# luotuoqingshan/SDPLRPlus.jl

Hardware: NVIDIA B200
Metric: AL inner iterations per second, MaxCut on a synthetic 10M-vertex power-law graph (rank 10) (higher is better)
Workload: dtype f64

## Files before the change

### sdplrplus.jl_b200/csrc/aop.cu

```cuda
#include <algorithm>
#include "common.cuh"

namespace {

constexpr int TPB = 256;

template <int VEC>
struct Ld;
template <>
struct Ld<1> {
    typedef double T;
    static __device__ __forceinline__ T ld(const double *p) { return __ldg(p); }
    static __device__ __forceinline__ double dot(T a, T b) { return a * b; }
};
template <>
struct Ld<2> {
    typedef double2 T;
    static __device__ __forceinline__ T ld(const double *p) { return ldg2(p); }
    static __device__ __forceinline__ double dot(T a, T b) { return a.x * b.x + a.y * b.y; }
};

template <int MODE, int VEC>
__device__ __forceinline__ void entry_accum(const double *__restrict__ U, const double *__restrict__ V, int r, int nv,
                                            int row, int col, int lg, int G, double v2, double &a1, double &a2,
// ... 73 lines not shown
    }
}

template <int MODE, int VEC>
__global__ void __launch_bounds__(TPB) k_A_rowc(long long lo, long long hi, const int *__restrict__ rowc_ptr,
                                                const double *__restrict__ rowc_val,
                                                const double *__restrict__ U, const double *__restrict__ V, int r, int G,
                                                double *__restrict__ out1, double *__restrict__ out2) {
    typedef Ld<VEC> L;
    __shared__ double sh1[TPB], sh2[TPB];
    const int nv = r / VEC;
    const int rpt = TPB / nv;
    const int rl = threadIdx.x / nv, c = threadIdx.x - rl * nv;
    const long long n_rows = hi - lo;
    for (long long t0 = (long long)blockIdx.x * rpt; t0 < n_rows; t0 += (long long)gridDim.x * rpt) {
        const long long i = lo + t0 + rl;
        const bool live = rl < rpt && i < hi;
        double d1 = 0.0, d2 = 0.0;
        int beg = 0, end = 0;
        if (live && c == 0) { beg = rowc_ptr[i]; end = rowc_ptr[i + 1]; }
        if (live) {
            typename L::T a = L::ld(U + (size_t)i * r + c * VEC);
            if (MODE == 0) {
                d1 = L::dot(a, a);
            } else {
                typename L::T b = L::ld(V + (size_t)i * r + c * VEC);
                d1 = L::dot(a, b);
                if (MODE == 2) d2 = L::dot(b, b);
            }
        }
        sh1[threadIdx.x] = d1;
        if (MODE == 2) sh2[threadIdx.x] = d2;
        __syncthreads();
        if (live && c == 0) {
            if (end > beg) {
                double s1 = 0.0, s2 = 0.0;
                for (int k = 0; k < nv; k++) { s1 += sh1[threadIdx.x + k]; if (MODE == 2) s2 += sh2[threadIdx.x + k]; }
                for (int k = beg; k < end; k++) {
                    const double val = rowc_val[k];
                    out1[k] = (MODE == 2 ? 2.0 : 1.0) * val * s1;
                    if (MODE == 2) out2[k] = val * s2;
                }
            }
        }
        __syncthreads();
    }
}

constexpr int kRowcUnroll = 4;
template <int MODE, int VEC>
__global__ void __launch_bounds__(TPB, 4) k_A_rowc_warp(long long lo, long long hi, const int *__restrict__ rowc_ptr,
// ... 8 lines not shown
    const bool act = rl < rpw;
    const long long n_rows = hi - lo;
    const long long per_trip = (long long)rpw * kRowcUnroll;
    const long long warp = (long long)blockIdx.x * (TPB / 32) + (threadIdx.x >> 5);
    const long long n_warps = (long long)gridDim.x * (TPB / 32);
    for (long long t0 = warp * per_trip; t0 < n_rows; t0 += n_warps * per_trip) {
        double d1[kRowcUnroll], d2[kRowcUnroll];
        int beg[kRowcUnroll], end[kRowcUnroll];
        typename L::T a[kRowcUnroll], b[kRowcUnroll];
#pragma unroll
        for (int u = 0; u < kRowcUnroll; u++) {
            const long long i = lo + t0 + (long long)u * rpw + rl;
            const bool live = act && i < hi;
            const long long is = live ? i : hi - 1;
            beg[u] = 0; end[u] = 0;
            if (live && c == 0) { beg[u] = rowc_ptr[i]; end[u] = rowc_ptr[i + 1]; }
            a[u] = L::ld(U + (size_t)is * r + c * VEC);
            if (MODE != 0) b[u] = L::ld(V + (size_t)is * r + c * VEC);
        }
#pragma unroll
        for (int u = 0; u < kRowcUnroll; u++) {
            d2[u] = 0.0;
            if (MODE == 0) {
                d1[u] = L::dot(a[u], a[u]);
            } else {
                d1[u] = L::dot(a[u], b[u]);
                if (MODE == 2) d2[u] = L::dot(b[u], b[u]);
            }
        }
#pragma unroll
        for (int u = 0; u < kRowcUnroll; u++) {
            double s1 = 0.0 + d1[u], s2 = 0.0 + d2[u];
            for (int k = 1; k < nv; k++) {
                s1 += __shfl_down_sync(0xffffffffu, d1[u], k);
                if (MODE == 2) s2 += __shfl_down_sync(0xffffffffu, d2[u], k);
            }
            for (int k = beg[u]; k < end[u]; k++) {
                const double val = rowc_val[k];
                out1[k] = (MODE == 2 ? 2.0 : 1.0) * val * s1;
                if (MODE == 2) out2[k] = val * s2;
            }
        }
    }
}

template <int MODE, int VEC>
__global__ void __launch_bounds__(TPB) k_A_long(const int *__restrict__ chunk_mat, const int *__restrict__ long_mat,
                                                const int *__restrict__ long_chunk_ptr, const int *__restrict__ matptr,
                                                const int *__restrict__ ent_row, const int *__restrict__ ent_col,
                                                const double *__restrict__ ent_two, const double *__restrict__ U,
// ... 80 lines not shown
            double t = 0.0;
            for (unsigned bI = 0; bI < gridDim.x; bI++) t += __ldcg(&part[(size_t)bI * (r * s) + e]);
            out[e] = t;
        }
        if (threadIdx.x == 0) *ticket = 0u;
    }
}

__global__ void k_lr_trace(int r, int s, const double *__restrict__ UB, const double *__restrict__ VB,
                           const double *__restrict__ Dg, double mult, double *__restrict__ out, int gid) {
    double acc[1] = {0.0};
    for (int e = threadIdx.x; e < r * s; e += blockDim.x) acc[0] += UB[e] * VB[e] * Dg[e / r];
    block_sum<1>(acc);
    if (threadIdx.x == 0) out[gid] = acc[0] * mult;
}

int pick_group(int nv) {
    int G = 1;
    while (G < nv && G < 32) G <<= 1;
    return G;
}

template <int MODE>
int32_t run_sparse(sdplrp_handle *h, const double *U, const double *V, double *out1, double *out2, int skip_mat = -1) {
    if (h->nA <= 0) return SDPLRP_OK;
    cudaStream_t st = h->stream;
    const int r = h->r;
    const bool vec2 = (r % 2 == 0);
    const int nv = vec2 ? r / 2 : r;
    const int G = pick_group(nv);
    const int gpb = TPB / G;
    const int grid_short = grid_for(h->nA, gpb, 16 * kNumSM);
    const int lo = (int)h->row_lo, hi = (int)h->row_hi;
    const unsigned char *sdf = h->n_sd > 0 ? h->sd_flag : nullptr;
    if (h->nA - h->n_sd - h->n_long > 0) {
        if (vec2) k_A_short<MODE, 2><<<grid_short, TPB, 0, st>>>((int)h->nA, h->matptr, h->mat_gid, h->ent_row, h->ent_col, h->ent_two, U, V, r, G, out1, out2, lo, hi, skip_mat, sdf);
        else k_A_short<MODE, 1><<<grid_short, TPB, 0, st>>>((int)h->nA, h->matptr, h->mat_gid, h->ent_row, h->ent_col, h->ent_two, U, V, r, G, out1, out2, lo, hi, skip_mat, sdf);
        KLAUNCH(h);
    }
    if (h->n_sd > 0 && nv <= 32 && h->rowc_kernel == 1 && h->world == 1) {
        const int grid_rows = grid_for(h->row_hi - h->row_lo, (TPB / 32) * (32 / nv) * kRowcUnroll, 16 * kNumSM);
        if (vec2) k_A_rowc_warp<MODE, 2><<<grid_rows, TPB, 0, st>>>(h->row_lo, h->row_hi, h->rowc_ptr, h->rowc_val, U, V, r, out1, out2);
        else k_A_rowc_warp<MODE, 1><<<grid_rows, TPB, 0, st>>>(h->row_lo, h->row_hi, h->rowc_ptr, h->rowc_val, U, V, r, out1, out2);
        KLAUNCH(h);
    } else if (h->n_sd > 0) {
        const int grid_rows = grid_for(h->row_hi - h->row_lo, TPB / nv, 16 * kNumSM);
        if (vec2) k_A_rowc<MODE, 2><<<grid_rows, TPB, 0, st>>>(h->row_lo, h->row_hi, h->rowc_ptr, h->rowc_val, U, V, r, G, out1, out2);
        else k_A_rowc<MODE, 1><<<grid_rows, TPB, 0, st>>>(h->row_lo, h->row_hi, h->rowc_ptr, h->rowc_val, U, V, r, G, out1, out2);
        KLAUNCH(h);
    }
    if (h->n_chunks > 0) {
        if (vec2) k_A_long<MODE, 2><<<(int)h->n_chunks, TPB, 0, st>>>(h->chunk_mat, h->long_mat, h->long_chunk_ptr, h->matptr, h->ent_row, h->ent_col, h->ent_two, U, V, r, G, h->chunk_part, lo, hi, skip_mat);
        else k_A_long<MODE, 1><<<(int)h->n_chunks, TPB, 0, st>>>(h->chunk_mat, h->long_mat, h->long_chunk_ptr, h->matptr, h->ent_row, h->ent_col, h->ent_two, U, V, r, G, h->chunk_part, lo, hi, skip_mat);
        KLAUNCH(h);
        k_A_long_combine<MODE><<<(int)h->n_long, TPB, 0, st>>>(h->long_mat, h->long_chunk_ptr, h->mat_gid, h->chunk_part, out1, out2, skip_mat);
        KLAUNCH(h);
    }
    CUDA_TRY(h, cudaGetLastError());
    return SDPLRP_OK;
}

}

int32_t lr_project(sdplrp_handle *h, const LowRank &L, const double *X, double *dst) {
    const int r = h->r;
    if (r > TPB) return fail(h, SDPLRP_ERR_ARG, "low-rank path supports r <= 256");
    const i64 lo = h->row_lo, nloc = h->row_hi - h->row_lo;
    for (i64 k0 = 0; k0 < L.s; k0 += kLrS) {
// ... 40 lines not shown
    }
    CUDA_TRY(h, cudaGetLastError());
    return SDPLRP_OK;
}

int32_t aop_uu_skip(sdplrp_handle *h, const double *U, double *out, bool skip_objective) {
    CUDA_TRY(h, cudaMemsetAsync(out, 0, (size_t)(h->m + 1) * sizeof(double), h->stream));
    SDP_CHECK(run_sparse<0>(h, U, nullptr, out, nullptr, skip_objective ? h->obj_mat : -1));
    return run_lowrank(h, 0, U, nullptr, out, nullptr);
}

int32_t aop_uu(sdplrp_handle *h, const double *U, double *out) { return aop_uu_skip(h, U, out, false); }

int32_t aop_uv(sdplrp_handle *h, const double *U, const double *V, double *out) {
    CUDA_TRY(h, cudaMemsetAsync(out, 0, (size_t)(h->m + 1) * sizeof(double), h->stream));
    SDP_CHECK(run_sparse<1>(h, U, V, out, nullptr));
    return run_lowrank(h, 1, U, V, out, nullptr);
}

int32_t aop_linesearch(sdplrp_handle *h, bool skip_objective) {
    const i64 z0 = h->world == 1 ? h->n_sd : 0;
    CUDA_TRY(h, cudaMemsetAsync(h->A_RD + z0, 0, (size_t)(h->m + 1 - z0) * sizeof(double), h->stream));
    CUDA_TRY(h, cudaMemsetAsync(h->A_DD + z0, 0, (size_t)(h->m + 1 - z0) * sizeof(double), h->stream));
    SDP_CHECK(run_sparse<2>(h, h->R, h->D, h->A_RD, h->A_DD, skip_objective ? h->obj_mat : -1));
    return run_lowrank(h, 2, h->R, h->D, h->A_RD, h->A_DD);
}
```

### sdplrplus.jl_b200/csrc/api.cu

```cuda
#include <math.h>
#include <stdlib.h>
#include <string.h>
#include <algorithm>
#include "common.cuh"

static const char *kNoHandle = "null handle";

#define REQUIRE_H(h) \
    if (!(h)) return SDPLRP_ERR_ARG
#define REQUIRE_PRE(h)                                                                   \
    if (!(h)->preprocessed) return fail(h, SDPLRP_ERR_STATE, "call sdplrp_preprocess first")
#define REQUIRE_RANK(h)                                                                  \
    if ((h)->r <= 0) return fail(h, SDPLRP_ERR_STATE, "call sdplrp_set_rank first")

int32_t fetch_scalars(sdplrp_handle *h, int first, int count) {
    CUDA_TRY(h, cudaMemcpyAsync(h->hscal + first, h->dscal + first, (size_t)count * sizeof(double), cudaMemcpyDeviceToHost, h->stream));
    CUDA_TRY(h, cudaStreamSynchronize(h->stream));
    return SDPLRP_OK;
}

cudaEvent_t prof_begin(sdplrp_handle *h) {
    cudaEvent_t e = nullptr;
    if (!h->ev_free.empty()) { e = h->ev_free.back(); h->ev_free.pop_back(); }
    else if (cudaEventCreate(&e) != cudaSuccess) return nullptr;
// ... 667 lines not shown
    REQUIRE_H(h); REQUIRE_PRE(h); REQUIRE_RANK(h);
    CUDA_TRY(h, cudaSetDevice(h->device));
    SDP_CHECK(lb_neg_copy(h));
    h->gram_g_valid = false;
    h->CD_valid = false; h->ls_valid = false;
    comm_mark_partial(h, SDPLRP_MAT_D);
    return SDPLRP_OK;
}

int32_t api_linesearch_coeffs_descent(sdplrp_handle *h, double bq[5], double *descent) {
    REQUIRE_H(h); REQUIRE_PRE(h); REQUIRE_RANK(h);
    CUDA_TRY(h, cudaSetDevice(h->device));
    const bool split = h->obj_mat >= 0;
    if (split && !h->CR_valid) SDP_CHECK(rebuild_CR(h));
    if (halo_active(h)) SDP_CHECK(halo_begin(h, h->D));
    else SDP_CHECK(comm_require_full(h, SDPLRP_MAT_D));
    if (needs_remote_R_rows(h)) SDP_CHECK(comm_require_full(h, SDPLRP_MAT_R));
    {
        SectionScope sc(h, SDPLRP_SEC_LS_PASS);
        SDP_CHECK(aop_linesearch(h, split));
    }
    if (split) {
        SectionScope sc(h, SDPLRP_SEC_SPMM);
        SDP_CHECK(grad_obj_spmm(h, h->D, h->CD, h->CR, h->dscal + SC_SUMS));
        SDP_CHECK(grad_obj_slots(h, h->dscal + SC_SUMS, h->A_RD + h->m, h->A_DD + h->m));
        h->CD_valid = true;
    }
    SDP_CHECK(comm_reduce_mvec(h, h->A_RD, h->A_DD));
    {
        SectionScope sc(h, SDPLRP_SEC_LS_COEFF);
        SDP_CHECK(vec_biquadratic(h));
    }
    h->ls_valid = true;
    static_assert(SC_DESCENT < SC_BQ, "one contiguous fetch covers descent and the coefficients");
    SDP_CHECK(fetch_scalars(h, SC_DESCENT, SC_BQ + 5 - SC_DESCENT));
    for (int k = 0; k < 5; k++) bq[k] = h->hscal[SC_BQ + k];
    if (descent) *descent = h->hscal[SC_DESCENT];
    return SDPLRP_OK;
}

int32_t sdplrp_linesearch_coeffs(sdplrp_handle *h, double bq[5]) { return api_linesearch_coeffs_descent(h, bq, nullptr); }


int32_t sdplrp_step(sdplrp_handle *h, double alpha, double *obj) {
    REQUIRE_H(h); REQUIRE_PRE(h); REQUIRE_RANK(h);
    CUDA_TRY(h, cudaSetDevice(h->device));
    {
// ... 220 lines not shown
```

### sdplrplus.jl_b200/csrc/common.cuh

```cuda
#pragma once
#include <cuda_runtime.h>
#include <stdint.h>
#include <algorithm>
#include <string>
#include <vector>
#include "../../include/sdplrp_b200.h"

typedef long long i64;

constexpr int kNumSM = 148;
constexpr int kMaxHist = 32;
constexpr int kRedBlocks = 4 * kNumSM;
constexpr int kRedThreads = 256;
constexpr int kMaxRedK = 64;
constexpr int kLbSmallLen = 17 * 17 + 3 * 17 + 17 + 7;
constexpr long long kPartialsLen = (long long)kRedBlocks * kMaxRedK * 8;
constexpr int kLongMatThreshold = 64;
constexpr int kChunkEntries = 2048;
constexpr int kRowGroupMax = 64;
constexpr int kRowWarpMax = 512;

static inline bool rank_supported(long long r) {
    return r >= 1 && r <= SDPLRP_MAX_RANK && (r % 2 == 0 || r <= SDPLRP_MAX_ODD_RANK);
}
// ... 296 lines not shown
        unsigned t = atomicAdd(ticket, 1u);
        is_last = (t == gridDim.x - 1);
    }
    __syncthreads();
    if (is_last) {
        __threadfence();
        double s[K];
#pragma unroll
        for (int k = 0; k < K; k++) s[k] = 0.0;
        for (unsigned bI = threadIdx.x; bI < gridDim.x; bI += blockDim.x) {
#pragma unroll
            for (int k = 0; k < K; k++) s[k] += __ldcg(&partials[(size_t)bI * K + k]);
        }
        block_sum<K>(s);
        if (threadIdx.x == 0) {
            fin(s);
            *ticket = 0u;
        }
    }
}

__device__ __forceinline__ double2 ldg2(const double *p) { return __ldg(reinterpret_cast<const double2 *>(p)); }

int32_t pre_build(sdplrp_handle *h, i64 n, i64 m, i64 nA, const int64_t *mat_off, const int64_t *I,
                  const int64_t *J, const double *V, const int64_t *gids, bool triplets_on_device = false);
int32_t pre_export(sdplrp_handle *h, int64_t *triu_colptr, int64_t *triu_rowval, int64_t *matptr,
                   int64_t *nzind, double *one, double *two, int64_t *full_colptr, int64_t *full_rowval,
                   int64_t *mapped);
void pre_free(sdplrp_handle *h);
void round_free(sdplrp_handle *h);

int32_t aop_uu(sdplrp_handle *h, const double *U, double *out_dev);
int32_t aop_uv(sdplrp_handle *h, const double *U, const double *V, double *out_dev);
int32_t aop_linesearch(sdplrp_handle *h, bool skip_objective);
int32_t aop_uu_skip(sdplrp_handle *h, const double *U, double *out_dev, bool skip_objective);

int32_t lr_project(sdplrp_handle *h, const LowRank &L, const double *X, double *dst);
int32_t lr_scratch(sdplrp_handle *h);

int32_t grad_form_y(sdplrp_handle *h);
int32_t grad_assemble_S(sdplrp_handle *h);
int32_t grad_spmm(sdplrp_handle *h, const double *X, double *Y, double scale, bool want_norm);
int32_t grad_spmm_sparse(sdplrp_handle *h, const double *X, double *Y, double scale);
int32_t grad_obj_spmm(sdplrp_handle *h, const double *X, double *Y, const double *Z, double *sums6);
inline bool obj_value_free(const sdplrp_handle *h) { return h->obj_value_free && h->vf_val != 0.0; }
int32_t grad_obj_slots(sdplrp_handle *h, const double *sums6, double *a_rd_m, double *a_dd_m);
int32_t grad_hot(sdplrp_handle *h);
int32_t grad_step_fused(sdplrp_handle *h, double alpha);
int32_t vec_tail_rest(sdplrp_handle *h, double alpha, const double *raw_in, double *raw_out, double *pn2_out);
int32_t grad_spmv(sdplrp_handle *h, const double *x, double *y, i64 ncols);
int32_t grad_triuS(sdplrp_handle *h, double *out_dev);

bool gather_supported(const sdplrp_handle *h);
int gather_tile_size(const sdplrp_handle *h);
void gather_plan_free(GatherPlan &p);
int32_t gather_plan_build(sdplrp_handle *h, GatherPlan &p, const int *ptr_dev, i64 row_lo, i64 row_hi, int T);
int32_t gather_spmm(sdplrp_handle *h, const GatherPlan &plan, const int *ptr, const int *idx, const double *val, const double *Xg,
                    const double *X, const double *Z, double *Y, int epi, double scale, double *sums4);

i64 tile_hot_rows(const sdplrp_handle *h);

int32_t vec_f_finish(sdplrp_handle *h);
int32_t vec_biquadratic(sdplrp_handle *h);
int32_t vec_commit(sdplrp_handle *h, double alpha);
int32_t vec_pnorm2(sdplrp_handle *h);
int32_t vec_dual_update(sdplrp_handle *h);
int32_t vec_armijo(sdplrp_handle *h, const double *alphas, int k, double *L, double *slope);
// ... 64 lines not shown
```

### sdplrplus.jl_b200/csrc/gradient.cu

```cuda
#include <algorithm>
#include "common.cuh"

namespace {

constexpr int TPB = 256;

__device__ __forceinline__ unsigned long long pol_evict_last() {
    unsigned long long p;
    asm volatile("createpolicy.fractional.L2::evict_last.b64 %0, 1.0;" : "=l"(p));
    return p;
}
__device__ __forceinline__ unsigned long long pol_evict_first() {
    unsigned long long p;
    asm volatile("createpolicy.fractional.L2::evict_first.b64 %0, 1.0;" : "=l"(p));
    return p;
}
__device__ __forceinline__ int ldg_i32_hint(const int *p, unsigned long long pol) {
    int v;
    asm volatile("ld.global.nc.L2::cache_hint.b32 %0, [%1], %2;" : "=r"(v) : "l"(p), "l"(pol));
    return v;
}
__device__ __forceinline__ double ldg_f64_hint(const double *p, unsigned long long pol) {
    double v;
    asm volatile("ld.global.nc.L2::cache_hint.f64 %0, [%1], %2;" : "=d"(v) : "l"(p), "l"(pol));
// ... 116 lines not shown
    const int *rows;
    i64 n_rows;
    const int *ptr, *idx;
    const int *beg_arr, *end_arr;
    const double *val;
    const int *src;
    const double *X;
    double *Y;
    int r, G;
    int Gw;
    int G0;
    int hot_rows;
    double scale, yobj;
    const double *ADD, *Z;
    double *partials;
    unsigned *ticket;
    double *out;
    i64 own_lo, own_hi;
    const int *chunk_start, *chunk_end, *chunk_row;
    const int *long_rows, *long_cptr;
    double *scratch;
    const double *vf_diag;
    double vf_scale;
};

template <int VEC, int MAXU, int EPI, bool VF = false>
__device__ __forceinline__ void row_epilogue(const RowArgs &a, i64 i, Acc<VEC> (&acc)[MAXU], int lg, int nv, double &s0, double &s1,
                                             int G) {
#pragma unroll
    for (int u = 0; u < MAXU; u++) {
        const int c = lg + u * G;
        if (c < nv) {
            const size_t off = (size_t)i * a.r + c * VEC;
            if (VF) acc[u].scale(a.vf_scale);
            if (EPI == 0) {
                acc[u].scale(a.scale);
            } else if (EPI == 3) {
                acc[u].accumulate_onto(a.scale, a.Y + off);
            } else if (EPI == 4) {
                acc[u].accumulate_onto(1.0, a.Y + off);
                s0 += acc[u].dot_ld(a.X + off);
                if (a.Z) {
                    Acc<VEC> t;
                    t.zero(); t.fma(1.0, a.X + off);
                    s1 += t.dot_ld(a.Z + off);
                }
            } else if (EPI == 1) {
                if (a.ADD) acc[u].scale_add(a.scale, a.yobj, a.ADD + off); else acc[u].scale(a.scale);
                s0 += acc[u].norm2();
            } else {
                s0 += acc[u].dot_ld(a.X + off);
                if (a.Z) {
                    Acc<VEC> t;
                    t.zero(); t.fma(1.0, a.X + off);
                    s1 += t.dot_ld(a.Z + off);
                }
            }
            acc[u].store(a.Y + off);
        }
    }
}

template <int EPI>
__device__ __forceinline__ void finish_sums(const RowArgs &a, double s0, double s1) {
    if (EPI == 0 || EPI == 3) return;
    double v[2] = {s0, s1};
    double *out = a.out;
    grid_sum_finalize<2>(v, a.partials, a.ticket, [&](double (&s)[2]) { out[0] = s[0]; out[1] = s[1]; });
}

#define VAL_AT(k) (IND ? __ldg(a.val + __ldg(a.src + (k))) : __ldg(a.val + (k)))

#ifndef SDPLRP_LB_GROUP
#define SDPLRP_LB_GROUP 0
#endif
#ifndef SDPLRP_LB_WARP
#define SDPLRP_LB_WARP 0
#endif
#if SDPLRP_LB_GROUP > 0
#define LB_GROUP __launch_bounds__(TPB, SDPLRP_LB_GROUP)
#else
#define LB_GROUP __launch_bounds__(TPB)
#endif
#if SDPLRP_LB_WARP > 0
#define LB_WARP __launch_bounds__(TPB, SDPLRP_LB_WARP)
#else
#define LB_WARP __launch_bounds__(TPB)
#endif

template <int VEC, int MAXU, bool IND, int EPI, int NB, bool VF>
__global__ void __launch_bounds__(TPB, VF && MAXU == 1 ? 4 : SDPLRP_LB_GROUP) k_rows_group(RowArgs a) {
    const int nv = a.r / VEC;
    const int G = a.G0;
    const int gpb = TPB / G;
    const int gib = threadIdx.x / G;
    const int lg = threadIdx.x - gib * G;
    const bool lane_ok = gib < gpb;
    const i64 group = (i64)blockIdx.x * gpb + gib;
    const i64 n_groups = (i64)gridDim.x * gpb;
    const unsigned long long p_hot = pol_evict_last(), p_str = pol_evict_first();
    double s0 = 0.0, s1 = 0.0;
    if (lane_ok)
    for (i64 q = group; q < a.n_rows; q += n_groups) {
        const i64 i = a.rows ? a.rows[q] : q;
        if (i < a.own_lo || i >= a.own_hi) continue;
        const int beg = a.beg_arr ? a.beg_arr[i] : a.ptr[i], end = a.end_arr ? a.end_arr[i] : a.ptr[i + 1];
        const double dii = VF ? a.vf_diag[i] : 0.0;
        Acc<VEC> acc[MAXU];
#pragma unroll
        for (int u = 0; u < MAXU; u++) acc[u].zero();
        for (int k0 = beg; k0 < end; k0 += NB) {
            int cc[NB];
            double vv[NB];
// ... 5 lines not shown
                else vv[j] = ok ? (IND ? __ldg(a.val + ldg_i32_hint(a.src + k0 + j, p_str)) : ldg_f64_hint(a.val + k0 + j, p_str)) : 0.0;
            }
#pragma unroll
            for (int u = 0; u < MAXU; u++) {
                const int c = lg + u * G;
                if (c < nv) {
                    if (VF) {
                        Acc<VEC> x[NB];
#pragma unroll
                        for (int j = 0; j < NB; j++) {
                            x[j].zero();
                            if (k0 + j < end) x[j].ld_hint(a.X + (size_t)cc[j] * a.r + c * VEC, cc[j] < a.hot_rows ? p_hot : p_str);
                        }
#pragma unroll
                        for (int j = 0; j < NB; j++) acc[u].fma_reg(vv[j], x[j]);
                    } else {
#pragma unroll
                        for (int j = 0; j < NB; j++)
                            if (k0 + j < end) acc[u].fma_hint(vv[j], a.X + (size_t)cc[j] * a.r + c * VEC, cc[j] < a.hot_rows ? p_hot : p_str);
                    }
                }
            }
        }
        row_epilogue<VEC, MAXU, EPI, VF>(a, i, acc, lg, nv, s0, s1, G);
    }
    finish_sums<EPI>(a, s0, s1);
}

template <int VEC, int MAXU, bool IND, int EPI, bool CHUNK, bool VF>
__global__ void LB_WARP k_rows_warp(RowArgs a) {
    const int nv = a.r / VEC;
    const int lane = threadIdx.x & 31;
    const int Gw = a.Gw, ng = 32 / Gw;
    const int grp = lane / Gw, lg = lane - grp * Gw;
    const bool lane_ok = grp < ng;
    const i64 warp = (i64)blockIdx.x * (TPB / 32) + (threadIdx.x >> 5);
    const i64 n_warps = (i64)gridDim.x * (TPB / 32);
    const unsigned long long p_hot = pol_evict_last(), p_str = pol_evict_first();
    double s0 = 0.0, s1 = 0.0;
    for (i64 q = warp; q < a.n_rows; q += n_warps) {
        const i64 i = CHUNK ? a.chunk_row[q] : (a.rows ? a.rows[q] : q);
        if (i < a.own_lo || i >= a.own_hi) continue;
        const int beg = CHUNK ? a.chunk_start[q] : (a.beg_arr ? a.beg_arr[i] : a.ptr[i]);
        const int end = CHUNK ? a.chunk_end[q] : (a.end_arr ? a.end_arr[i] : a.ptr[i + 1]);
        const double dii = VF ? a.vf_diag[i] : 0.0;
        Acc<VEC> acc[MAXU];
#pragma unroll
        for (int u = 0; u < MAXU; u++) acc[u].zero();
        for (int k0 = beg + grp * 4; lane_ok && k0 < end; k0 += ng * 4) {
            int cc[4];
            double vv[4];
#pragma unroll
// ... 24 lines not shown
                }
            }
        }
        if ((Gw & (Gw - 1)) == 0) {
#pragma unroll
            for (int u = 0; u < MAXU; u++)
                for (int o = Gw; o < 32; o <<= 1) acc[u].shfl_add(o);
        } else {
#pragma unroll
            for (int u = 0; u < MAXU; u++) {
                const Acc<VEC> own = acc[u];
                for (int o = 1; o < ng; o++) acc[u].add_from_lane(own, (((lane_ok ? grp : 0) + o) % ng) * Gw + lg);
            }
        }
        if (grp == 0) {
            if (CHUNK) {
#pragma unroll
                for (int u = 0; u < MAXU; u++) {
                    const int c = lg + u * Gw;
                    if (c < nv) acc[u].store(a.scratch + (size_t)q * a.r + c * VEC);
                }
            } else {
                row_epilogue<VEC, MAXU, EPI, VF>(a, i, acc, lg, nv, s0, s1, Gw);
            }
        }
    }
    if (!CHUNK) finish_sums<EPI>(a, s0, s1);
}

template <int VEC, int MAXU, int EPI, bool VF>
__global__ void __launch_bounds__(TPB) k_rows_combine(RowArgs a) {
    const int nv = a.r / VEC;
    const int lg = threadIdx.x & (a.G - 1);
    const i64 group = ((i64)blockIdx.x * TPB + threadIdx.x) / a.G;
    const i64 n_groups = (i64)gridDim.x * TPB / a.G;
    double s0 = 0.0, s1 = 0.0;
    for (i64 q = group; q < a.n_rows; q += n_groups) {
        const i64 i = a.long_rows[q];
        if (i < a.own_lo || i >= a.own_hi) continue;
        Acc<VEC> acc[MAXU];
#pragma unroll
        for (int u = 0; u < MAXU; u++) acc[u].zero();
        for (int c = a.long_cptr[q]; c < a.long_cptr[q + 1]; c++) {
#pragma unroll
            for (int u = 0; u < MAXU; u++) {
                const int p = lg + u * a.G;
                if (p < nv) acc[u].add_mem(a.scratch + (size_t)c * a.r + p * VEC);
            }
        }
        row_epilogue<VEC, MAXU, EPI, VF>(a, i, acc, lg, nv, s0, s1, a.G);
    }
    finish_sums<EPI>(a, s0, s1);
}

__global__ void k_lr_apply(i64 lo, i64 hi, int r, int s, i64 n, const double *__restrict__ XB, const double *__restrict__ Dg,
                           const double *__restrict__ B, const double *__restrict__ y, int gid, double scale,
                           double *__restrict__ Y) {
    const double coeff = scale * y[gid];
    for (i64 e = lo * r + blockIdx.x * (i64)blockDim.x + threadIdx.x; e < hi * r; e += (i64)gridDim.x * blockDim.x) {
        const i64 j = e / r;
        const int i = (int)(e - j * r);
        double t = 0.0;
        for (int k = 0; k < s; k++) t += XB[k * r + i] * Dg[k] * __ldg(&B[j + k * n]);
        Y[e] += coeff * t;
    }
}

constexpr int SPMV_L = 8;
__global__ void __launch_bounds__(TPB) k_spmv(i64 n, const int *__restrict__ ptr, const int *__restrict__ idx,
                                              const double *__restrict__ S, const double *__restrict__ x,
                                              double *__restrict__ y) {
    const int lg = threadIdx.x & (SPMV_L - 1);
    const i64 warp_global = (i64)blockIdx.x * (TPB / 32) + (threadIdx.x >> 5);
// ... 147 lines not shown
    const int *ptr, *idx;
    const double *val;
    const int *src;
    const RowClasses *cls;
};

static int32_t classes_fork(sdplrp_handle *h) {
    if (!h->class_streams[0]) return SDPLRP_OK;
    CUDA_TRY(h, cudaEventRecord(h->ev_fork, h->stream));
    for (int c = 0; c < 2; c++) CUDA_TRY(h, cudaStreamWaitEvent(h->class_streams[c], h->ev_fork, 0));
    h->fork_open = true;
    return SDPLRP_OK;
}
static int32_t classes_join(sdplrp_handle *h) {
    if (!h->class_streams[0]) return SDPLRP_OK;
    for (int c = 0; c < 2; c++) {
        CUDA_TRY(h, cudaEventRecord(h->ev_join[c], h->class_streams[c]));
        CUDA_TRY(h, cudaStreamWaitEvent(h->stream, h->ev_join[c], 0));
    }
    h->fork_open = false;
    return SDPLRP_OK;
}

template <int VEC, int MAXU, bool IND, int EPI, bool VF>
int32_t launch_classes(sdplrp_handle *h, RowArgs a, const RowClasses &cls, const TileLayout &longs, double *sums ,
                       bool long_empty = false, int class_mask = 7) {
    const int gpb = TPB / a.G;
    const int gpb0 = TPB / a.G0;
    const int spmm_cap = 16 * kNumSM;
    const bool fork = h->class_streams[0] != nullptr;
    const bool own_fork = fork && !h->fork_open;
    if (own_fork) SDP_CHECK(classes_fork(h));
    for (int c = 0; c < 3; c++) {
        if (!(class_mask & (1 << c))) continue;
        cudaStream_t st = (fork && c > 0) ? h->class_streams[c - 1] : h->stream;
        if (sums) a.out = sums + 2 * c;
        a.partials = h->partials + (size_t)c * 16384;
        a.ticket = h->ticket + c;
        a.rows = cls.list[c];
        a.n_rows = cls.cnt[c];
        if (a.n_rows <= 0) {
            if (sums) CUDA_TRY(h, cudaMemsetAsync(sums + 2 * c, 0, 2 * sizeof(double), st));
            continue;
        }
        if (c == 0) {
            if (h->spmm_unroll >= 8) k_rows_group<VEC, MAXU, IND, EPI, 8, VF><<<grid_for(a.n_rows, gpb0, spmm_cap), TPB, 0, st>>>(a);
            else k_rows_group<VEC, MAXU, IND, EPI, 4, VF><<<grid_for(a.n_rows, gpb0, spmm_cap), TPB, 0, st>>>(a);
        } else if (c == 1) {
            k_rows_warp<VEC, MAXU, IND, EPI, false, VF><<<grid_for(a.n_rows, TPB / 32, spmm_cap), TPB, 0, st>>>(a);
        } else if (long_empty) {
            RowArgs b = a;
            b.beg_arr = a.ptr + 1; b.end_arr = a.ptr + 1;
            k_rows_warp<VEC, MAXU, IND, EPI, false, VF><<<grid_for(b.n_rows, TPB / 32, spmm_cap), TPB, 0, st>>>(b);
        } else {
            const i64 need = longs.n_chunks * (i64)a.r;
            if (h->tile_scratch_len < need) {
                if (fork) CUDA_TRY(h, cudaDeviceSynchronize());
                SDP_CHECK(dev_alloc(h, &h->tile_scratch, need));
                h->tile_scratch_len = need;
            }
            RowArgs b = a;
            b.chunk_start = longs.chunk_start; b.chunk_end = longs.chunk_end; b.chunk_row = longs.chunk_row;
            b.long_rows = longs.long_rows; b.long_cptr = longs.long_cptr; b.scratch = h->tile_scratch;
            b.n_rows = longs.n_chunks;
            k_rows_warp<VEC, MAXU, IND, EPI, true, VF><<<grid_for(b.n_rows, TPB / 32, spmm_cap), TPB, 0, st>>>(b);
            KLAUNCH(h);
            b.n_rows = longs.n_long;
            k_rows_combine<VEC, MAXU, EPI, VF><<<grid_for(b.n_rows, gpb, 4 * kNumSM), TPB, 0, st>>>(b);
        }
        KLAUNCH(h);
    }
    if (own_fork) SDP_CHECK(classes_join(h));
    CUDA_TRY(h, cudaGetLastError());
    return SDPLRP_OK;
}

template <bool IND, int EPI, bool VF = false>
int32_t launch_csr(sdplrp_handle *h, RowArgs a, const RowClasses &cls, const TileLayout &longs, double *sums, bool long_empty = false,
                   i64 hot_override = -1, int class_mask = 7) {
    const int r = h->r;
    const bool vec2 = (r % 2 == 0);
    const int nv = vec2 ? r / 2 : r;
    a.r = r;
    a.G = pick_group(nv);
    if (a.own_hi <= 0) {
        a.own_lo = h->row_lo;
        a.own_hi = h->row_hi;
    }
    a.G0 = (nv <= 32 && h->spmm_g0) ? nv : a.G;
    a.hot_rows = (int)(hot_override >= 0 ? hot_override : tile_hot_rows(h));
    const int units = (nv + a.G - 1) / a.G;
    a.Gw = (h->spmm_g0 && nv <= 16 && units == 1) ? nv : a.G;
    if (units > 4) return fail(h, SDPLRP_ERR_ARG, "rank too large for the sparse kernels (r <= 256 even / 128 odd)");
    if (vec2) {
        if (units == 1) return launch_classes<2, 1, IND, EPI, VF>(h, a, cls, longs, sums, long_empty, class_mask);
        return launch_classes<2, 4, IND, EPI, VF>(h, a, cls, longs, sums, long_empty, class_mask);
    }
    if (units == 1) return launch_classes<1, 1, IND, EPI, VF>(h, a, cls, longs, sums, long_empty, class_mask);
    return launch_classes<1, 4, IND, EPI, VF>(h, a, cls, longs, sums, long_empty, class_mask);
}

__global__ void k_row_split(i64 n, const int *__restrict__ ptr, const int *__restrict__ idx, int hub_cols, int *__restrict__ mid) {
    for (i64 i = blockIdx.x * (i64)blockDim.x + threadIdx.x; i < n; i += (i64)gridDim.x * blockDim.x) {
        int lo = ptr[i], hi = ptr[i + 1];
        while (lo < hi) {
            const int m = lo + ((hi - lo) >> 1);
            if (idx[m] < hub_cols) lo = m + 1; else hi = m;
        }
        mid[i] = lo;
    }
}

static i64 phase_hub_cols(const sdplrp_handle *h) {
    if (h->spmm_phases <= 0 || !h->relabeled || h->dealt || h->world > 1 || h->nnzF <= 0) return 0;
    const i64 want = h->spmm_phases == 1 ? (i64)(64.0 * 1024 * 1024) / (8 * (i64)std::max(1, h->r)) : (i64)h->spmm_phases;
    return std::min<i64>(want, h->n);
}
static int32_t ensure_row_mid(sdplrp_handle *h, i64 hub_cols) {
    if (h->row_mid && h->row_mid_cols == hub_cols) return SDPLRP_OK;
    SDP_CHECK(dev_alloc(h, &h->row_mid, h->n));
    k_row_split<<<grid_for(h->n, TPB, 8 * kNumSM), TPB, 0, h->stream>>>(h->n, h->full_ptr, h->full_idx, (int)hub_cols, h->row_mid);
    KLAUNCH(h);
    CUDA_TRY(h, cudaGetLastError());
    h->row_mid_cols = hub_cols;
    return SDPLRP_OK;
}

int32_t add_lowrank(sdplrp_handle *h, const double *X, double *Y, double scale) {
    if (h->lr.empty()) return SDPLRP_OK;
    const int r = h->r;
    SDP_CHECK(lr_scratch(h));
    for (const LowRank &L : h->lr) {
        SDP_CHECK(lr_project(h, L, X, h->lr_tmp));
        k_lr_apply<<<grid_for((h->row_hi - h->row_lo) * r, TPB, kRedBlocks), TPB, 0, h->stream>>>(
            h->row_lo, h->row_hi, r, (int)L.s, h->n, h->lr_tmp, L.dD, L.dB, h->y, (int)L.gid, scale, Y);
        KLAUNCH(h);
    }
    CUDA_TRY(h, cudaGetLastError());
    return SDPLRP_OK;
}

}

int32_t grad_form_y(sdplrp_handle *h) {
    k_form_y<<<grid_for(h->m + 1, TPB, kRedBlocks), TPB, 0, h->stream>>>(h->m, h->sigma, h->lambda, h->lambda_ub, h->pvio_raw, h->y);
    KLAUNCH(h);
    h->y_obj = 1.0;
    h->S_current = false;
    CUDA_TRY(h, cudaGetLastError());
// ... 76 lines not shown
        const double hidden = std::min(std::max(0.0, exch - ls - 0.1), 0.58 * 1.27 * sweep);
        const double extra = 0.33 * sweep + 0.1;
        single_sweep = hidden < extra + 0.15;
    }
    if (single_sweep) {
        SDP_CHECK(halo_wait(h, 0));
        SDP_CHECK(halo_wait(h, 1));
        return launch_csr<false, 2>(h, a, p.cls, p.longs, sums6);
    }
    SDP_CHECK(halo_wait(h, 0));
    RowArgs a1 = a;
    a1.end_arr = p.lmid;
    SDP_CHECK((launch_csr<false, 0>(h, a1, p.cls, p.longs, nullptr, false, -1, 3)));
    SDP_CHECK(halo_wait(h, 1));
    RowArgs a2 = a;
    a2.beg_arr = p.lmid;
    SDP_CHECK(classes_fork(h));
    int32_t rc = launch_csr<false, 4>(h, a2, p.cls, p.longs, sums6, false, -1, 3);
    if (rc == SDPLRP_OK) rc = launch_csr<false, 2>(h, a, p.cls, p.longs, sums6, false, -1, 4);
    const int32_t rj = classes_join(h);
    return rc != SDPLRP_OK ? rc : rj;
}

int32_t grad_obj_spmm(sdplrp_handle *h, const double *X, double *Y, const double *Z, double *sums6) {
    if (halo_active(h)) return grad_obj_spmm_halo(h, X, Y, Z, sums6);
    if (gather_supported(h) && h->nnzF > 0) {
        SDP_CHECK(gather_plan_build(h, h->full_plan, h->full_ptr, h->row_lo, h->row_hi, gather_tile_size(h)));
        CUDA_TRY(h, cudaMemsetAsync(sums6 + 4, 0, 2 * sizeof(double), h->stream));
        return gather_spmm(h, h->full_plan, h->full_ptr, h->full_idx, h->Cfull, X, X, Z, Y, 2, 1.0, sums6);
    }
    RowArgs a = {};
    a.ptr = h->full_ptr; a.idx = h->full_idx; a.val = h->Cfull; a.src = nullptr;
    a.X = X; a.Y = Y; a.Z = Z; a.scale = 1.0;
    const i64 hub_cols = phase_hub_cols(h);
    if (hub_cols > 0 && hub_cols < h->n) {
        SDP_CHECK(ensure_row_mid(h, hub_cols));
        a.end_arr = h->row_mid;
        SDP_CHECK((launch_csr<false, 0>(h, a, h->full_cls, h->full_long, nullptr, false, hub_cols)));
        a.beg_arr = h->row_mid; a.end_arr = nullptr;
        return launch_csr<false, 4>(h, a, h->full_cls, h->full_long, sums6, true, hub_cols);
    }
    if (obj_value_free(h)) {
        a.val = nullptr; a.vf_diag = h->vf_diag; a.vf_scale = h->vf_val;
        return launch_csr<false, 2, true>(h, a, h->full_cls, h->full_long, sums6);
    }
    return launch_csr<false, 2>(h, a, h->full_cls, h->full_long, sums6);
}

int32_t grad_hot(sdplrp_handle *h) {
    cudaStream_t st = h->stream;
    const int r = h->r;
    const bool need_dynS = h->n_dyn > 0 && h->n_dyn_nsd > 0;
    if (need_dynS) {
        k_S_dynamic<2><<<grid_for(h->n_dyn, TPB, 8 * kNumSM), TPB, 0, st>>>(h->n_dyn, 0.0, h->dyn_slot, h->dyn_ptr, h->dyn_nsd_end, h->dyn_gid, h->dyn_val,
                                                                           h->dyn_pos_a, h->dyn_pos_b, h->triuS_static, h->y, h->dynS);
        KLAUNCH(h);
    }
    const bool vec2 = (r % 2 == 0);
    const int nv = vec2 ? r / 2 : r;
    const i64 total = (h->row_hi - h->row_lo) * nv;
    const double *CR = (h->obj_mat >= 0) ? h->CR : nullptr;
    const int grid = grid_for(total, TPB * 2, kRedBlocks);
    if (vec2) k_grad_diag<2><<<grid, TPB, 0, st>>>(h->row_lo, h->row_hi, r, h->y_obj, CR, h->R, h->rowc_ptr, h->rowc_val, h->y, h->dyn_diag, need_dynS ? h->dynS : nullptr, h->G, h->partials, h->ticket, h->dscal + SC_GNORM2);
    else k_grad_diag<1><<<grid, TPB, 0, st>>>(h->row_lo, h->row_hi, r, h->y_obj, CR, h->R, h->rowc_ptr, h->rowc_val, h->y, h->dyn_diag, need_dynS ? h->dynS : nullptr, h->G, h->partials, h->ticket, h->dscal + SC_GNORM2);
    KLAUNCH(h);
    bool renorm = false;
    if (h->n_dynF > 0) {
        RowArgs a = {};
// ... 97 lines not shown
```

Measured before the change: 126.9.

## Fold line-search row-constraint dot products into objective SpMM pass

During line search, the per-row constraint values A(R·D) and A(D·D) for diagonal (row-list) constraints are now computed inside the objective SpMM kernels, which already stream D. The separate rowc kernel launch is skipped for this case. The goal is to save one full pass over R and D plus a launch. It adds a ROWC template variant with extra loads and shuffles in the row kernels, and swaps the dot helpers for explicit rounding intrinsics.

```diff
diff --git a/sdplrplus.jl_b200/csrc/aop.cu b/sdplrplus.jl_b200/csrc/aop.cu
--- a/sdplrplus.jl_b200/csrc/aop.cu
+++ b/sdplrplus.jl_b200/csrc/aop.cu
@@ -119,11 +119,11 @@
         if (live) {
             typename L::T a = L::ld(U + (size_t)i * r + c * VEC);
             if (MODE == 0) {
-                d1 = L::dot(a, a);
+                d1 = piece_dot(a, a);
             } else {
                 typename L::T b = L::ld(V + (size_t)i * r + c * VEC);
-                d1 = L::dot(a, b);
-                if (MODE == 2) d2 = L::dot(b, b);
+                d1 = piece_dot(a, b);
+                if (MODE == 2) d2 = piece_dot(b, b);
             }
         }
         sh1[threadIdx.x] = d1;
@@ -178,10 +178,10 @@
         for (int u = 0; u < kRowcUnroll; u++) {
             d2[u] = 0.0;
             if (MODE == 0) {
-                d1[u] = L::dot(a[u], a[u]);
+                d1[u] = piece_dot(a[u], a[u]);
             } else {
-                d1[u] = L::dot(a[u], b[u]);
-                if (MODE == 2) d2[u] = L::dot(b[u], b[u]);
+                d1[u] = piece_dot(a[u], b[u]);
+                if (MODE == 2) d2[u] = piece_dot(b[u], b[u]);
             }
         }
 #pragma unroll
@@ -308,7 +308,8 @@
 }
 
 template <int MODE>
-int32_t run_sparse(sdplrp_handle *h, const double *U, const double *V, double *out1, double *out2, int skip_mat = -1) {
+int32_t run_sparse(sdplrp_handle *h, const double *U, const double *V, double *out1, double *out2, int skip_mat = -1,
+                   bool skip_rowc = false) {
     if (h->nA <= 0) return SDPLRP_OK;
     cudaStream_t st = h->stream;
     const int r = h->r;
@@ -324,12 +325,13 @@
         else k_A_short<MODE, 1><<<grid_short, TPB, 0, st>>>((int)h->nA, h->matptr, h->mat_gid, h->ent_row, h->ent_col, h->ent_two, U, V, r, G, out1, out2, lo, hi, skip_mat, sdf);
         KLAUNCH(h);
     }
-    if (h->n_sd > 0 && nv <= 32 && h->rowc_kernel == 1 && h->world == 1) {
+    const bool rowc = h->n_sd > 0 && !skip_rowc;
+    if (rowc && nv <= 32 && h->rowc_kernel == 1 && h->world == 1) {
         const int grid_rows = grid_for(h->row_hi - h->row_lo, (TPB / 32) * (32 / nv) * kRowcUnroll, 16 * kNumSM);
         if (vec2) k_A_rowc_warp<MODE, 2><<<grid_rows, TPB, 0, st>>>(h->row_lo, h->row_hi, h->rowc_ptr, h->rowc_val, U, V, r, out1, out2);
         else k_A_rowc_warp<MODE, 1><<<grid_rows, TPB, 0, st>>>(h->row_lo, h->row_hi, h->rowc_ptr, h->rowc_val, U, V, r, out1, out2);
         KLAUNCH(h);
-    } else if (h->n_sd > 0) {
+    } else if (rowc) {
         const int grid_rows = grid_for(h->row_hi - h->row_lo, TPB / nv, 16 * kNumSM);
         if (vec2) k_A_rowc<MODE, 2><<<grid_rows, TPB, 0, st>>>(h->row_lo, h->row_hi, h->rowc_ptr, h->rowc_val, U, V, r, G, out1, out2);
         else k_A_rowc<MODE, 1><<<grid_rows, TPB, 0, st>>>(h->row_lo, h->row_hi, h->rowc_ptr, h->rowc_val, U, V, r, G, out1, out2);
@@ -416,6 +418,6 @@
     const i64 z0 = h->world == 1 ? h->n_sd : 0;
     CUDA_TRY(h, cudaMemsetAsync(h->A_RD + z0, 0, (size_t)(h->m + 1 - z0) * sizeof(double), h->stream));
     CUDA_TRY(h, cudaMemsetAsync(h->A_DD + z0, 0, (size_t)(h->m + 1 - z0) * sizeof(double), h->stream));
-    SDP_CHECK(run_sparse<2>(h, h->R, h->D, h->A_RD, h->A_DD, skip_objective ? h->obj_mat : -1));
+    SDP_CHECK(run_sparse<2>(h, h->R, h->D, h->A_RD, h->A_DD, skip_objective ? h->obj_mat : -1, skip_objective && ls_rowc_fold(h)));
     return run_lowrank(h, 2, h->R, h->D, h->A_RD, h->A_DD);
 }
diff --git a/sdplrplus.jl_b200/csrc/api.cu b/sdplrplus.jl_b200/csrc/api.cu
--- a/sdplrplus.jl_b200/csrc/api.cu
+++ b/sdplrplus.jl_b200/csrc/api.cu
@@ -713,7 +713,7 @@
     }
     if (split) {
         SectionScope sc(h, SDPLRP_SEC_SPMM);
-        SDP_CHECK(grad_obj_spmm(h, h->D, h->CD, h->CR, h->dscal + SC_SUMS));
+        SDP_CHECK(grad_obj_spmm(h, h->D, h->CD, h->CR, h->dscal + SC_SUMS, true));
         SDP_CHECK(grad_obj_slots(h, h->dscal + SC_SUMS, h->A_RD + h->m, h->A_DD + h->m));
         h->CD_valid = true;
     }
diff --git a/sdplrplus.jl_b200/csrc/common.cuh b/sdplrplus.jl_b200/csrc/common.cuh
--- a/sdplrplus.jl_b200/csrc/common.cuh
+++ b/sdplrplus.jl_b200/csrc/common.cuh
@@ -342,6 +342,9 @@
 
 __device__ __forceinline__ double2 ldg2(const double *p) { return __ldg(reinterpret_cast<const double2 *>(p)); }
 
+__device__ __forceinline__ double piece_dot(double a, double b) { return __dmul_rn(a, b); }
+__device__ __forceinline__ double piece_dot(double2 a, double2 b) { return __fma_rn(a.x, b.x, __dmul_rn(a.y, b.y)); }
+
 int32_t pre_build(sdplrp_handle *h, i64 n, i64 m, i64 nA, const int64_t *mat_off, const int64_t *I,
                   const int64_t *J, const double *V, const int64_t *gids, bool triplets_on_device = false);
 int32_t pre_export(sdplrp_handle *h, int64_t *triu_colptr, int64_t *triu_rowval, int64_t *matptr,
@@ -362,7 +365,8 @@
 int32_t grad_assemble_S(sdplrp_handle *h);
 int32_t grad_spmm(sdplrp_handle *h, const double *X, double *Y, double scale, bool want_norm);
 int32_t grad_spmm_sparse(sdplrp_handle *h, const double *X, double *Y, double scale);
-int32_t grad_obj_spmm(sdplrp_handle *h, const double *X, double *Y, const double *Z, double *sums6);
+int32_t grad_obj_spmm(sdplrp_handle *h, const double *X, double *Y, const double *Z, double *sums6, bool line_search = false);
+bool ls_rowc_fold(const sdplrp_handle *h);
 inline bool obj_value_free(const sdplrp_handle *h) { return h->obj_value_free && h->vf_val != 0.0; }
 int32_t grad_obj_slots(sdplrp_handle *h, const double *sums6, double *a_rd_m, double *a_dd_m);
 int32_t grad_hot(sdplrp_handle *h);
diff --git a/sdplrplus.jl_b200/csrc/gradient.cu b/sdplrplus.jl_b200/csrc/gradient.cu
--- a/sdplrplus.jl_b200/csrc/gradient.cu
+++ b/sdplrplus.jl_b200/csrc/gradient.cu
@@ -162,6 +162,10 @@
     double *scratch;
     const double *vf_diag;
     double vf_scale;
+    const double *rowc_R;
+    const int *rowc_ptr;
+    const double *rowc_val;
+    double *rowc_out1, *rowc_out2;
 };
 
 template <int VEC, int MAXU, int EPI, bool VF = false>
@@ -201,6 +205,57 @@
     }
 }
 
+template <int VEC>
+__device__ __forceinline__ void rowc_piece(const RowArgs &a, i64 i, int c, double &d1, double &d2) {
+    const size_t off = (size_t)i * a.r + c * VEC;
+    if (VEC == 2) {
+        const double2 u = ldg2(a.rowc_R + off), v = ldg2(a.X + off);
+        d1 = piece_dot(u, v); d2 = piece_dot(v, v);
+    } else {
+        const double u = __ldg(a.rowc_R + off), v = __ldg(a.X + off);
+        d1 = piece_dot(u, v); d2 = piece_dot(v, v);
+    }
+}
+__device__ __forceinline__ void rowc_store(const RowArgs &a, int beg, int end, double s1, double s2) {
+    for (int p = beg; p < end; p++) {
+        const double val = a.rowc_val[p];
+        a.rowc_out1[p] = 2.0 * val * s1;
+        a.rowc_out2[p] = val * s2;
+    }
+}
+constexpr int kRowcFoldUnroll = 2;
+template <int VEC>
+__device__ __forceinline__ void rowc_fold(const RowArgs &a, i64 i, int nv) {
+    const int beg = a.rowc_ptr[i], end = a.rowc_ptr[i + 1];
+    if (beg >= end) return;
+    double s1 = 0.0, s2 = 0.0;
+#pragma unroll kRowcFoldUnroll
+    for (int c = 0; c < nv; c++) {
+        double d1, d2;
+        rowc_piece<VEC>(a, i, c, d1, d2);
+        s1 += d1; s2 += d2;
+    }
+    rowc_store(a, beg, end, s1, s2);
+}
+template <int VEC>
+__device__ __forceinline__ void rowc_fold_group(const RowArgs &a, i64 i, int lg, int nv, int G, double d1, double d2, int beg,
+                                                int end) {
+    const int lane = threadIdx.x & 31;
+    const int first = lane - lg;
+    const int lo = max(first, 0), hi = min(first + G, 32);
+    const unsigned mask = hi - lo == 32 ? 0xffffffffu : ((1u << (hi - lo)) - 1u) << lo;
+    double s1 = 0.0 + d1, s2 = 0.0 + d2;
+    for (int k = 1; k < nv; k++) {
+        const int src = min(max(first + k, lo), hi - 1);
+        double t1 = __shfl_sync(mask, d1, src), t2 = __shfl_sync(mask, d2, src);
+        if (lg == 0) {
+            if (first + k >= 32) rowc_piece<VEC>(a, i, k, t1, t2);
+            s1 += t1; s2 += t2;
+        }
+    }
+    if (lg == 0) rowc_store(a, beg, end, s1, s2);
+}
+
 template <int EPI>
 __device__ __forceinline__ void finish_sums(const RowArgs &a, double s0, double s1) {
     if (EPI == 0 || EPI == 3) return;
@@ -228,7 +283,7 @@
 #define LB_WARP __launch_bounds__(TPB)
 #endif
 
-template <int VEC, int MAXU, bool IND, int EPI, int NB, bool VF>
+template <int VEC, int MAXU, bool IND, int EPI, int NB, bool VF, bool ROWC>
 __global__ void __launch_bounds__(TPB, VF && MAXU == 1 ? 4 : SDPLRP_LB_GROUP) k_rows_group(RowArgs a) {
     const int nv = a.r / VEC;
     const int G = a.G0;
@@ -280,12 +335,19 @@
                 }
             }
         }
+        double f1 = 0.0, f2 = 0.0;
+        int fbeg = 0, fend = 0;
+        if (ROWC) {
+            if (lg < nv) rowc_piece<VEC>(a, i, lg, f1, f2);
+            if (lg == 0) { fbeg = a.rowc_ptr[i]; fend = a.rowc_ptr[i + 1]; }
+        }
         row_epilogue<VEC, MAXU, EPI, VF>(a, i, acc, lg, nv, s0, s1, G);
+        if (ROWC) rowc_fold_group<VEC>(a, i, lg, nv, G, f1, f2, fbeg, fend);
     }
     finish_sums<EPI>(a, s0, s1);
 }
 
-template <int VEC, int MAXU, bool IND, int EPI, bool CHUNK, bool VF>
+template <int VEC, int MAXU, bool IND, int EPI, bool CHUNK, bool VF, bool ROWC>
 __global__ void LB_WARP k_rows_warp(RowArgs a) {
     const int nv = a.r / VEC;
     const int lane = threadIdx.x & 31;
@@ -356,13 +418,14 @@
                 }
             } else {
                 row_epilogue<VEC, MAXU, EPI, VF>(a, i, acc, lg, nv, s0, s1, Gw);
+                if (ROWC && lg == 0) rowc_fold<VEC>(a, i, nv);
             }
         }
     }
     if (!CHUNK) finish_sums<EPI>(a, s0, s1);
 }
 
-template <int VEC, int MAXU, int EPI, bool VF>
+template <int VEC, int MAXU, int EPI, bool VF, bool ROWC>
 __global__ void __launch_bounds__(TPB) k_rows_combine(RowArgs a) {
     const int nv = a.r / VEC;
     const int lg = threadIdx.x & (a.G - 1);
@@ -383,6 +446,7 @@
             }
         }
         row_epilogue<VEC, MAXU, EPI, VF>(a, i, acc, lg, nv, s0, s1, a.G);
+        if (ROWC && lg == 0) rowc_fold<VEC>(a, i, nv);
     }
     finish_sums<EPI>(a, s0, s1);
 }
@@ -576,7 +640,7 @@
     return SDPLRP_OK;
 }
 
-template <int VEC, int MAXU, bool IND, int EPI, bool VF>
+template <int VEC, int MAXU, bool IND, int EPI, bool VF, bool ROWC>
 int32_t launch_classes(sdplrp_handle *h, RowArgs a, const RowClasses &cls, const TileLayout &longs, double *sums ,
                        bool long_empty = false, int class_mask = 7) {
     const int gpb = TPB / a.G;
@@ -598,14 +662,14 @@
             continue;
         }
         if (c == 0) {
-            if (h->spmm_unroll >= 8) k_rows_group<VEC, MAXU, IND, EPI, 8, VF><<<grid_for(a.n_rows, gpb0, spmm_cap), TPB, 0, st>>>(a);
-            else k_rows_group<VEC, MAXU, IND, EPI, 4, VF><<<grid_for(a.n_rows, gpb0, spmm_cap), TPB, 0, st>>>(a);
+            if (h->spmm_unroll >= 8) k_rows_group<VEC, MAXU, IND, EPI, 8, VF, ROWC><<<grid_for(a.n_rows, gpb0, spmm_cap), TPB, 0, st>>>(a);
+            else k_rows_group<VEC, MAXU, IND, EPI, 4, VF, ROWC><<<grid_for(a.n_rows, gpb0, spmm_cap), TPB, 0, st>>>(a);
         } else if (c == 1) {
-            k_rows_warp<VEC, MAXU, IND, EPI, false, VF><<<grid_for(a.n_rows, TPB / 32, spmm_cap), TPB, 0, st>>>(a);
+            k_rows_warp<VEC, MAXU, IND, EPI, false, VF, ROWC><<<grid_for(a.n_rows, TPB / 32, spmm_cap), TPB, 0, st>>>(a);
         } else if (long_empty) {
             RowArgs b = a;
             b.beg_arr = a.ptr + 1; b.end_arr = a.ptr + 1;
-            k_rows_warp<VEC, MAXU, IND, EPI, false, VF><<<grid_for(b.n_rows, TPB / 32, spmm_cap), TPB, 0, st>>>(b);
+            k_rows_warp<VEC, MAXU, IND, EPI, false, VF, ROWC><<<grid_for(b.n_rows, TPB / 32, spmm_cap), TPB, 0, st>>>(b);
         } else {
             const i64 need = longs.n_chunks * (i64)a.r;
             if (h->tile_scratch_len < need) {
@@ -617,10 +681,10 @@
             b.chunk_start = longs.chunk_start; b.chunk_end = longs.chunk_end; b.chunk_row = longs.chunk_row;
             b.long_rows = longs.long_rows; b.long_cptr = longs.long_cptr; b.scratch = h->tile_scratch;
             b.n_rows = longs.n_chunks;
-            k_rows_warp<VEC, MAXU, IND, EPI, true, VF><<<grid_for(b.n_rows, TPB / 32, spmm_cap), TPB, 0, st>>>(b);
+            k_rows_warp<VEC, MAXU, IND, EPI, true, VF, false><<<grid_for(b.n_rows, TPB / 32, spmm_cap), TPB, 0, st>>>(b);
             KLAUNCH(h);
             b.n_rows = longs.n_long;
-            k_rows_combine<VEC, MAXU, EPI, VF><<<grid_for(b.n_rows, gpb, 4 * kNumSM), TPB, 0, st>>>(b);
+            k_rows_combine<VEC, MAXU, EPI, VF, ROWC><<<grid_for(b.n_rows, gpb, 4 * kNumSM), TPB, 0, st>>>(b);
         }
         KLAUNCH(h);
     }
@@ -629,7 +693,7 @@
     return SDPLRP_OK;
 }
 
-template <bool IND, int EPI, bool VF = false>
+template <bool IND, int EPI, bool VF = false, bool ROWC = false>
 int32_t launch_csr(sdplrp_handle *h, RowArgs a, const RowClasses &cls, const TileLayout &longs, double *sums, bool long_empty = false,
                    i64 hot_override = -1, int class_mask = 7) {
     const int r = h->r;
@@ -646,12 +710,13 @@
     const int units = (nv + a.G - 1) / a.G;
     a.Gw = (h->spmm_g0 && nv <= 16 && units == 1) ? nv : a.G;
     if (units > 4) return fail(h, SDPLRP_ERR_ARG, "rank too large for the sparse kernels (r <= 256 even / 128 odd)");
-    if (vec2) {
-        if (units == 1) return launch_classes<2, 1, IND, EPI, VF>(h, a, cls, longs, sums, long_empty, class_mask);
-        return launch_classes<2, 4, IND, EPI, VF>(h, a, cls, longs, sums, long_empty, class_mask);
-    }
-    if (units == 1) return launch_classes<1, 1, IND, EPI, VF>(h, a, cls, longs, sums, long_empty, class_mask);
-    return launch_classes<1, 4, IND, EPI, VF>(h, a, cls, longs, sums, long_empty, class_mask);
+    if (units == 1) {
+        if (vec2) return launch_classes<2, 1, IND, EPI, VF, ROWC>(h, a, cls, longs, sums, long_empty, class_mask);
+        return launch_classes<1, 1, IND, EPI, VF, ROWC>(h, a, cls, longs, sums, long_empty, class_mask);
+    }
+    if constexpr (ROWC) return fail(h, SDPLRP_ERR_ARG, "row-list fold of the gather pass needs one unit per row");
+    else if (vec2) return launch_classes<2, 4, IND, EPI, VF, false>(h, a, cls, longs, sums, long_empty, class_mask);
+    else return launch_classes<1, 4, IND, EPI, VF, false>(h, a, cls, longs, sums, long_empty, class_mask);
 }
 
 __global__ void k_row_split(i64 n, const int *__restrict__ ptr, const int *__restrict__ idx, int hub_cols, int *__restrict__ mid) {
@@ -679,6 +744,17 @@
     h->row_mid_cols = hub_cols;
     return SDPLRP_OK;
 }
+
+}
+
+bool ls_rowc_fold(const sdplrp_handle *h) {
+    const int nv = h->r % 2 == 0 ? h->r / 2 : h->r;
+    const i64 hub_cols = phase_hub_cols(h);
+    return h->world == 1 && h->obj_mat >= 0 && h->n_sd > 0 && h->rowc_kernel == 1 && nv <= 32 &&
+           !(gather_supported(h) && h->nnzF > 0) && !(hub_cols > 0 && hub_cols < h->n);
+}
+
+namespace {
 
 int32_t add_lowrank(sdplrp_handle *h, const double *X, double *Y, double scale) {
     if (h->lr.empty()) return SDPLRP_OK;
@@ -801,7 +877,7 @@
     return rc != SDPLRP_OK ? rc : rj;
 }
 
-int32_t grad_obj_spmm(sdplrp_handle *h, const double *X, double *Y, const double *Z, double *sums6) {
+int32_t grad_obj_spmm(sdplrp_handle *h, const double *X, double *Y, const double *Z, double *sums6, bool line_search) {
     if (halo_active(h)) return grad_obj_spmm_halo(h, X, Y, Z, sums6);
     if (gather_supported(h) && h->nnzF > 0) {
         SDP_CHECK(gather_plan_build(h, h->full_plan, h->full_ptr, h->row_lo, h->row_hi, gather_tile_size(h)));
@@ -819,10 +895,17 @@
         a.beg_arr = h->row_mid; a.end_arr = nullptr;
         return launch_csr<false, 4>(h, a, h->full_cls, h->full_long, sums6, true, hub_cols);
     }
+    const bool fold = line_search && ls_rowc_fold(h);
+    if (fold) {
+        a.rowc_R = h->R; a.rowc_ptr = h->rowc_ptr; a.rowc_val = h->rowc_val;
+        a.rowc_out1 = h->A_RD; a.rowc_out2 = h->A_DD;
+    }
     if (obj_value_free(h)) {
         a.val = nullptr; a.vf_diag = h->vf_diag; a.vf_scale = h->vf_val;
+        if (fold) return launch_csr<false, 2, true, true>(h, a, h->full_cls, h->full_long, sums6);
         return launch_csr<false, 2, true>(h, a, h->full_cls, h->full_long, sums6);
     }
+    if (fold) return launch_csr<false, 2, false, true>(h, a, h->full_cls, h->full_long, sums6);
     return launch_csr<false, 2>(h, a, h->full_cls, h->full_long, sums6);
 }
 
```

Result: slower. 123.1, median of 6 (-2.9%).
